# XiaRho/CMDA

Measured on AMD Instinct MI355X. Metric: training images/sec (512x512 image+event, MiT-B5), higher is better.
Workload: dtype bf16

## Files before the change

cmda_amd/_lib.py:

```python
import ctypes
import os

import torch

_HERE = os.path.dirname(os.path.abspath(__file__))
_LIB_PATH = os.environ.get('CMDA_HIP_LIB') or os.path.join(_HERE, 'libcmda_hip.so')

c_i32, c_i64, c_f32, c_vp = ctypes.c_int32, ctypes.c_int64, ctypes.c_float, ctypes.c_void_p

F32, BF16 = 0, 1
U8, I64 = 0, 1
ABI_VERSION, ABI_EXT_VERSION = 8, 1
ABI_EXT2_VERSION = 1
ABI_EXT3_VERSION = 1
ABI_EXT4_VERSION = 1
ABI_EXT5_VERSION = 1


class View(ctypes.Structure):
    _fields_ = [('ptr', c_vp), ('ld', c_i64), ('R', c_i64), ('Cc', c_i64), ('batch_stride', c_i64), ('batch2_stride', c_i64),
                ('conv', c_i32), ('H', c_i32), ('W', c_i32), ('C', c_i32), ('OH', c_i32), ('OW', c_i32),
                ('KH', c_i32), ('KW', c_i32), ('stride', c_i32), ('pad', c_i32), ('dil', c_i32),
                ('in_dil', c_i32), ('reflect', c_i32), ('vec_ok', c_i32)]


class GemmParams(ctypes.Structure):
    _fields_ = [('A', View), ('B', View), ('a_kstrided', c_i32), ('b_kstrided', c_i32), ('C', c_vp),
                ('ldc', c_i64), ('c_batch_stride', c_i64), ('c_batch2_stride', c_i64), ('M', c_i32), ('N', c_i32),
                ('K', c_i32), ('batch', c_i32), ('batch2', c_i32), ('splits', c_i32), ('alpha', c_f32), ('beta', c_f32), ('bias', c_vp),
                ('act', c_i32), ('res', c_vp), ('ldres', c_i64), ('res_batch_stride', c_i64), ('res_batch2_stride', c_i64),
                ('rowscale', c_vp), ('rows_per_scale', c_i32), ('out_f32', c_i32), ('atomic', c_i32),
                ('dtype', c_i32), ('c_vec_ok', c_i32), ('colsum', c_vp),
                ('c_patch_ow', c_i32), ('c_patch_kh', c_i32), ('c_patch_kwci', c_i32), ('tile_hint', c_i32), ('c_perm_ci', c_i32), ('c_perm_cells', c_i32),
                ('res_f32', c_i32), ('colstats_rows', c_i32), ('colstats', c_vp)]


class CmdaError(RuntimeError):
    pass


_ERR = {-1: 'bad shape', -2: 'unsupported dtype', -3: 'HIP launch error', -4: 'unsupported argument combination'}

_lib = None
_emulated = False


def _declare(lib):
    lib.cmda_abi_version.restype = ctypes.c_int
    lib.cmda_layernorm_bwd_ws_floats.restype = ctypes.c_int64
# ... 6 lines not shown
    if not hasattr(lib, 'cmdax_abi_version'):
        raise CmdaError('the kernel library lacks the ABI extension (cmdax_*): rebuild it')
    lib.cmdax_abi_version.restype = ctypes.c_int
    if lib.cmdax_abi_version() != ABI_EXT_VERSION:
        raise CmdaError('libcmda_hip.so ABI extension version mismatch')
    if not hasattr(lib, 'cmdax2_abi_version'):
        raise CmdaError('the kernel library lacks the second ABI table (cmdax2_*): rebuild it')
    lib.cmdax2_abi_version.restype = ctypes.c_int
    if lib.cmdax2_abi_version() != ABI_EXT2_VERSION:
        raise CmdaError('libcmda_hip.so second ABI table (cmdax2_*) version mismatch')
    if not hasattr(lib, 'cmdax3_abi_version'):
        raise CmdaError('the kernel library lacks the third ABI table (cmdax3_*): rebuild it')
    lib.cmdax3_abi_version.restype = ctypes.c_int
    if lib.cmdax3_abi_version() != ABI_EXT3_VERSION:
        raise CmdaError('libcmda_hip.so third ABI table (cmdax3_*) version mismatch')
    lib.cmdax3_sky_mask_ws_bytes.restype = ctypes.c_int64
    lib.cmdax3_sky_mask_ws_bytes.argtypes = [ctypes.c_int, ctypes.c_int, ctypes.c_int]
    if not hasattr(lib, 'cmdax4_abi_version'):
        raise CmdaError('the kernel library lacks the fourth ABI table (cmdax4_*): rebuild it')
    lib.cmdax4_abi_version.restype = ctypes.c_int
    if lib.cmdax4_abi_version() != ABI_EXT4_VERSION:
        raise CmdaError('libcmda_hip.so fourth ABI table (cmdax4_*) version mismatch')
    lib.cmdax4_cow_mask_ws_bytes.restype = ctypes.c_int64
    lib.cmdax4_cow_mask_ws_bytes.argtypes = [ctypes.c_int, ctypes.c_int, ctypes.c_int, ctypes.c_int]
    if not hasattr(lib, 'cmdax5_abi_version'):
        raise CmdaError('the kernel library lacks the fifth ABI table (cmdax5_*): rebuild it')
    lib.cmdax5_abi_version.restype = ctypes.c_int
    if lib.cmdax5_abi_version() != ABI_EXT5_VERSION:
        raise CmdaError('libcmda_hip.so fifth ABI table (cmdax5_*) version mismatch')
    lib.cmdax5_voxel_ordered_ws_bytes.restype = ctypes.c_int64
    lib.cmdax5_voxel_ordered_ws_bytes.argtypes = [ctypes.c_int, ctypes.c_int64, ctypes.c_int, ctypes.c_int, ctypes.c_int]
    lib.cmdax5_events_norm_ws_bytes.restype = ctypes.c_int64
    lib.cmdax5_events_norm_ws_bytes.argtypes = [ctypes.c_int, ctypes.c_int64]
    return lib


def _load():
    global _lib
    if _lib is not None:
        return _lib
    if not os.path.exists(_LIB_PATH):
        raise CmdaError(
            f'{_LIB_PATH} not found: build the gfx950 kernel library first '
            '(python -c "import __graft_entry__ as g; g.build()" or `make hip`). '
            'cmda_amd has no CPU fallback.')
    _lib = _declare(ctypes.CDLL(_LIB_PATH))
    if _lib.cmda_abi_version() != ABI_VERSION:
        raise CmdaError('libcmda_hip.so ABI version mismatch')
    return _lib


def _bind_for_tests(path):
    global _lib, _emulated
    _lib = _declare(ctypes.CDLL(path))
    _emulated = True
    return _lib


def _unbind_for_tests():
    global _lib, _emulated
    _lib = None
    _emulated = False


def emulated():
    return _emulated
# ... 55 lines not shown
```

cmda_amd/csrc/dwconv.hip:

```cpp
#include "common.h"
#include <cstdlib>

namespace {

struct RunGeom {
  int H, W, dil, rpc, rpr;
  long nruns;
};
static inline RunGeom run_geom(int B, int H, int W, int dil, int run) {
  RunGeom g;
  g.H = H; g.W = W; g.dil = dil;
  const int per_class = (W + dil - 1) / dil;
  g.rpc = (per_class + run - 1) / run;
  g.rpr = dil * g.rpc;
  g.nruns = (long)B * H * g.rpr;
  return g;
}

#ifdef CMDA_EMU
#define CMDA_DW_PIN(v) (void)(v)
#else
#define CMDA_DW_PIN(v) asm volatile("" : "+v"(v))
#endif
template <typename T> struct Raw;
template <> struct Raw<float> {
  float4 v;
  __device__ __forceinline__ void load(const float* p, bool ok) {
    v = *reinterpret_cast<const float4*>(p);
    if (!ok) v = make_float4(0.f, 0.f, 0.f, 0.f);
  }
  __device__ __forceinline__ void unpack(float (&o)[4]) const { o[0] = v.x; o[1] = v.y; o[2] = v.z; o[3] = v.w; }
};
template <> struct Raw<bf16_t> {
// ... 275 lines not shown
  for (int r = 0; r < RL; ++r) {
    const int gr = rgrp[r];
    if (gr >= 0) {
      if (g0 < 0) g0 = gr;
      else if (gr != g0) uniform = false;
    }
  }
  if (g0 < 0) return;
  const unsigned slot = (unsigned)blk.by & (CMDA_BN_SLOTS - 1);
  if (uniform) {
    if (py != 0) return;
    float* wsl = stats + ((long)g0 * (CMDA_BN_SLOTS + 1) + slot) * 2 * (long)C + c;
#pragma unroll
    for (int q = 0; q < 4; ++q) {
      float a = 0.f, b2 = 0.f;
#pragma unroll
      for (int r = 0; r < RL; ++r) {
        a += red[r][cx][q];
        b2 += red[r][cx][4 + q];
      }
      atomicAdd(wsl + q, a);
      atomicAdd(wsl + C + q, b2);
    }
  } else if (grp >= 0) {
    float* wsl = stats + ((long)grp * (CMDA_BN_SLOTS + 1) + slot) * 2 * (long)C + c;
#pragma unroll
    for (int q = 0; q < 4; ++q) {
      atomicAdd(wsl + q, cs[q]);
      atomicAdd(wsl + C + q, cq[q]);
    }
  }
}

template <int CQ>
static __device__ __forceinline__ void dw_fold_atomics(float (&red)[256 / CQ][CQ][41], const float (&acc)[9][4], const float (&accb)[4],
                                                       float* __restrict__ dw, float* __restrict__ dbias, int bx, int C) {
  constexpr int RL = 256 / CQ;
  const int cx = threadIdx.x % CQ, py = threadIdx.x / CQ;
  {
    float* slot = red[py][cx];
#pragma unroll
    for (int t = 0; t < 9; ++t)
#pragma unroll
      for (int j = 0; j < 4; ++j) slot[t * 4 + j] = acc[t][j];
#pragma unroll
    for (int j = 0; j < 4; ++j) slot[36 + j] = accb[j];
  }
  __syncthreads();
  for (int k = threadIdx.x; k < CQ * 40; k += blockDim.x) {
    const int gx = k / 40, v = k - gx * 40;
    const int cc = (bx * CQ + gx) * 4;
    if (cc >= C) continue;
    float s = 0.f;
#pragma unroll
    for (int l = 0; l < RL; ++l) s += red[l][gx][v];
    if (v < 36) {
      const int t = v >> 2, j = v & 3;
      atomicAdd(dw + (cc + j) * 9 + t, s);
    } else if (dbias) {
      atomicAdd(dbias + cc + (v - 36), s);
    }
  }
}

template <typename T, int CQ>
__global__ __launch_bounds__(256) void dw_bwd_weight_kernel(const T* __restrict__ dz, const T* __restrict__ x,
// ... 322 lines not shown
  if (npix * C <= 0) return CMDA_OK;
  if ((C & 3) || dil < 1) return CMDA_ERR_SHAPE;
  if (too_big(npix)) return CMDA_ERR_SHAPE;
  const int gx = (C / 4 + 63) / 64;
  if (dil >= 2 && MODE != 1 && (MODE == 2 || act == 0)) {
    DilGeom dg;
    dg.H = H; dg.W = W; dg.dil = dil;
    dg.rpc = ((W + dil - 1) / dil + DRUN - 1) / DRUN;
    dg.nthreads = (long)B * dil * dil * dg.rpc;
    constexpr int cq = 64;
    const long nb = (dg.nthreads + 256 / cq - 1) / (256 / cq) * gx;
    if (too_big(dg.nthreads) || nb > 0x7fffffffL) return CMDA_ERR_SHAPE;
    CMDA_DISPATCH_DTYPE(dtype, CMDA_LAUNCH((dw_dilated_kernel<T, MODE == 1 ? 0 : MODE, cq>), dim3((unsigned)nb), dim3(256), 0, stream,
                                           (const T*)x, w, bias, (T*)out, dg, C, act, accumulate, gx, stats, imgs_per_group));
    CMDA_CHECK_LAUNCH();
  }
  if (stats) return CMDA_ERR_UNSUPPORTED;
  if constexpr (MODE != 1) {
    int band;
    if (walk_takes<MODE>(B, H, W, C, dil, dtype, &band)) {
      const int rc = launch_walk<MODE, 64>(x, w, bias, da, out, nullptr, nullptr, B, H, W, C, act, accumulate, stream, band);
      if (rc != kWalkDeclined) return rc;
    }
  }
  const RunGeom g = run_geom(B, H, W, dil, run_len(dtype));
  if (too_big(g.nruns)) return CMDA_ERR_SHAPE;
  const long nblk = (g.nruns + 3) / 4 * gx;
  if (nblk > 0x7fffffffL) return CMDA_ERR_SHAPE;
  dim3 grid((unsigned)nblk);
  CMDA_DISPATCH_DTYPE(dtype, CMDA_LAUNCH((dw_stencil_kernel<T, MODE>), grid, dim3(256), 0, stream, (const T*)x, w, bias,
                                         (const T*)da, (T*)out, g, C, act, accumulate, gx));
  CMDA_CHECK_LAUNCH();
}
}

extern "C" int cmda_dwconv3x3_fwd(const void* x, const float* w, const float* bias, void* y, int B, int H, int W, int C,
                                  int dil, int act, int dtype, void* stream) {
  return launch_stencil<0>(x, w, bias, nullptr, y, B, H, W, C, dil, act, 0, dtype, stream);
}

extern "C" int cmda_dwconv3x3_fwd_stats(const void* x, const float* w, const float* bias, void* y, int B, int H, int W, int C,
                                        int dil, float* colstats, int imgs_per_group, int dtype, void* stream) {
  if (!colstats || imgs_per_group < 1 || B % imgs_per_group || dil < 2) return CMDA_ERR_UNSUPPORTED;
  return launch_stencil<0>(x, w, bias, nullptr, y, B, H, W, C, dil, 0, 0, dtype, stream, colstats, imgs_per_group);
}

extern "C" int cmda_dwconv3x3_gelu_bwd_prep(const void* x, const float* w, const float* bias, const void* da, void* dz,
                                            int B, int H, int W, int C, int dil, int dtype, void* stream) {
  return launch_stencil<1>(x, w, bias, da, dz, B, H, W, C, dil, 2, 0, dtype, stream);
}

extern "C" int cmda_dwconv3x3_bwd_data(const void* dy, const float* w, void* dx, int B, int H, int W, int C, int dil,
                                       int accumulate, int dtype, void* stream) {
  return launch_stencil<2>(dy, w, nullptr, nullptr, dx, B, H, W, C, dil, 0, accumulate, dtype, stream);
}

extern "C" int cmda_dwconv3x3_bwd_weight(const void* dz, const void* x, float* dw, float* dbias, int B, int H, int W,
                                         int C, int dil, int dtype, void* stream) {
  const long npix = (long)B * H * W;
  if (npix * C <= 0) return CMDA_OK;
  if ((C & 3) || dil < 1) return CMDA_ERR_SHAPE;
  const RunGeom g = run_geom(B, H, W, dil, run_len(dtype));
  if (too_big(npix) || too_big(g.nruns)) return CMDA_ERR_SHAPE;
  constexpr int cq = 16, rl = 256 / cq;
  const int gx = (C / 4 + cq - 1) / cq;
  int k = 8;
// ... 32 lines not shown
```

cmda_amd/decode_heads.py:

```python
import torch
import torch.nn as nn

from . import nn as K
from . import deferred, ops
from . import runtime as rt
from .registry import HEADS, LOSSES, build_loss


class ConvModule(nn.Module):

    def __init__(self, cin, cout, k, padding=0, dilation=1, groups=1, norm=True):
        super().__init__()
        self.conv = nn.Conv2d(cin, cout, k, padding=padding, dilation=dilation, groups=groups, bias=not norm)
        self.bn = nn.BatchNorm2d(cout) if norm else None
        nn.init.kaiming_normal_(self.conv.weight, a=0, mode='fan_out', nonlinearity='relu')
        if self.conv.bias is not None:
            nn.init.zeros_(self.conv.bias)
        self.k, self.padding, self.dilation, self.groups = k, padding, dilation, groups


class DepthwiseSeparableConvModule(nn.Module):
    def __init__(self, cin, cout, k, padding, dilation):
        super().__init__()
        self.depthwise_conv = ConvModule(cin, cin, k, padding=padding, dilation=dilation, groups=cin)
        self.pointwise_conv = ConvModule(cin, cout, 1)


class MLP(nn.Module):
    def __init__(self, input_dim=2048, embed_dim=768):
        super().__init__()
        self.proj = nn.Linear(input_dim, embed_dim)


def _bn_stats_ws(bn, dev, M, C, groups):
    if not bn.training or M % groups or not ops.colstats_ok(M // groups, C):
        return None
    return ops.bn_stats_ws(dev, groups, C)


def _bn_fwd(bn, x, y, M, C, relu, ldy=None, coff=0, groups=1, order=None, stats_ws=None):
    if bn.training:
        mean, rstd = ops.bn_train_fwd(x, bn.weight, bn.bias, y, bn.running_mean, bn.running_var, M // groups, C, bn.eps,
                                      bn.momentum, relu, ldy, coff, groups, order, stats_ws=stats_ws)
    else:
        mean, rstd = bn.running_mean, torch.rsqrt(bn.running_var + bn.eps)
        ops.bn_apply(x, mean, rstd, bn.weight, bn.bias, y, M, C, relu, ldy, coff)
        mean, rstd = mean.expand(groups, C).contiguous(), rstd.expand(groups, C).contiguous()
    return mean, rstd


def _bn_bwd(bn, dy, x, stats, M, C, relu, lddy=None, coff=0, groups=1):
    mean, rstd = stats
    return ops.bn_train_bwd(dy, x, mean, rstd, bn.weight, bn.bias, rt.grad(bn.weight), rt.grad(bn.bias), M // groups, C, relu,
                            lddy, coff, groups)


class ASPPWrapper(nn.Module):

    def __init__(self, in_channels, channels, sep, dilations, pool=False, norm_cfg=None, act_cfg=None,
                 align_corners=False, context_cfg=None):
        super().__init__()
        assert not pool and context_cfg is None, 'only the configuration CMDA uses is implemented'
        assert sep, 'CMDA uses the depthwise-separable ASPP'
        self.dilations = tuple(dilations)
        self.in_channels, self.channels = in_channels, channels
        mods = []
        for d in self.dilations:
            mods.append(ConvModule(in_channels, channels, 1) if d == 1 else
                        DepthwiseSeparableConvModule(in_channels, channels, 3, padding=d, dilation=d))
        self.aspp_modules = nn.ModuleList(mods)
        self.bottleneck = ConvModule(len(self.dilations) * channels, channels, 3, padding=1)

    def fwd(self, x, B, H, W, groups=1, order=None):
        M, Cin, Ch = B * H * W, self.in_channels, self.channels
        nb = len(self.dilations)
        cat = torch.empty(M, nb * Ch, dtype=rt.compute_dtype(), device=x.device)
        saved = []
        g = dict(groups=groups, order=order)
        for j, (d, m) in enumerate(zip(self.dilations, self.aspp_modules)):
            if d == 1:
                ws = _bn_stats_ws(m.bn, x.device, M, Ch, groups)
                z = K.linear_fwd(x, m.conv.weight, None, M, Cin, colstats=None if ws is None else (ws, M // groups))
                st = _bn_fwd(m.bn, z, cat, M, Ch, True, nb * Ch, j * Ch, stats_ws=ws, **g)
                saved.append((z, st))
            else:
                dwm, pwm = m.depthwise_conv, m.pointwise_conv
                ws = _bn_stats_ws(dwm.bn, x.device, M, Cin, groups) if (d >= 2 and B % groups == 0) else None
                u = ops.dwconv_fwd(x, rt.wdw(dwm.conv.weight), None, B, H, W, Cin, d, None, colstats=None if ws is None else (ws, B // groups))
                ub = torch.empty_like(u)
                st_u = _bn_fwd(dwm.bn, u, ub, M, Cin, True, stats_ws=ws, **g)
                ws = _bn_stats_ws(pwm.bn, x.device, M, Ch, groups)
                z = K.linear_fwd(ub, pwm.conv.weight, None, M, Cin, colstats=None if ws is None else (ws, M // groups))
                st_z = _bn_fwd(pwm.bn, z, cat, M, Ch, True, nb * Ch, j * Ch, stats_ws=ws, **g)
                saved.append((u, st_u, ub, z, st_z))
        ws = _bn_stats_ws(self.bottleneck.bn, x.device, M, Ch, groups)
        zb, _, _ = K.conv_fwd(cat, self.bottleneck.conv.weight, None, B, H, W, 1, 1, colstats=None if ws is None else (ws, M // groups))
        feat = torch.empty_like(zb)
        st_b = _bn_fwd(self.bottleneck.bn, zb, feat, M, Ch, True, stats_ws=ws, **g)
        return feat, (x, cat, saved, zb, st_b, groups)

    def bwd(self, sv, dfeat, B, H, W):
        x, cat, saved, zb, st_b, groups = sv
        M, Cin, Ch = B * H * W, self.in_channels, self.channels
        nb = len(self.dilations)
        dzb = _bn_bwd(self.bottleneck.bn, dfeat, zb, st_b, M, Ch, True, groups=groups)
        dcat = K.conv_bwd(dzb, cat, self.bottleneck.conv.weight, None, B, H, W, 1, 1)
        dx = torch.empty(M, Cin, dtype=rt.compute_dtype(), device=x.device)
        first = True
        for j, (d, m) in enumerate(zip(self.dilations, self.aspp_modules)):
            if d == 1:
                z, st = saved[j]
                dz = _bn_bwd(m.bn, dcat, z, st, M, Ch, True, nb * Ch, j * Ch, groups=groups)
                K.linear_bwd(dz, x, m.conv.weight, None, M, Cin, dx_out=dx, dx_beta=0.0 if first else 1.0)
            else:
                u, st_u, ub, z, st_z = saved[j]
                dwm, pwm = m.depthwise_conv, m.pointwise_conv
                dz = _bn_bwd(pwm.bn, dcat, z, st_z, M, Ch, True, nb * Ch, j * Ch, groups=groups)
                dub = K.linear_bwd(dz, ub, pwm.conv.weight, None, M, Cin)
                du = _bn_bwd(dwm.bn, dub, u, st_u, M, Cin, True, groups=groups)
                deferred.tail_defer(lambda du=du, gw=rt.grad(dwm.conv.weight).view(Cin, 9), d=d:
                                    ops.dwconv_bwd_weight(du, x, gw, None, B, H, W, Cin, d))
                ops.dwconv_bwd_data(du, rt.wdw(dwm.conv.weight), B, H, W, Cin, d, out=dx, accumulate=not first)
            first = False
        return dx


def build_layer(in_channels, out_channels, type, **kwargs):
    if type == 'id':
        return nn.Identity()
    if type == 'mlp':
        return MLP(input_dim=in_channels, embed_dim=out_channels)
    if type == 'aspp':
        return ASPPWrapper(in_channels=in_channels, channels=out_channels, **kwargs)
    raise NotImplementedError(type)


@LOSSES.register_module()
class CrossEntropyLoss(nn.Module):

    def __init__(self, use_sigmoid=False, use_mask=False, reduction='mean', class_weight=None, loss_weight=1.0):
        super().__init__()
        assert not use_sigmoid and not use_mask, 'only the softmax cross-entropy of configs/fusion/* is implemented'
        assert reduction == 'mean'
        self.use_sigmoid, self.use_mask, self.reduction = use_sigmoid, use_mask, reduction
        self.loss_weight, self.class_weight = loss_weight, class_weight


def ce_losses_fwd(logits, seg_label, seg_weight, ignore_index, loss_weight):
    B, _, H, W = seg_label.shape
    label = seg_label.view(B, H, W)
    wgt = seg_weight.float().contiguous() if seg_weight is not None else None
    acc, lse = ops.ce_upsample_fwd(logits, label, wgt, H, W, ignore_index)
    n = float(B * H * W)
    loss = acc[0] * (loss_weight / n)
    accuracy = acc[1:2] * (100.0 / n)
# ... 360 lines not shown
```

cmda_amd/ops.py:

```python
import ctypes
import os

import numpy as np
import torch

from . import _lib as L
from . import deferred as D
from ._lib import BF16, F32, GemmParams, View, c_f32, c_i32, c_i64, call, check_dev, dtype_tag, ptr, stream_of

_ESIZE = {torch.float32: 4, torch.bfloat16: 2}


def _chunk(t):
    return 16 // _ESIZE[t.dtype]


def plain_view(t, rows, cols, ld=None, batch_stride=0, offset=0, batch2_stride=0):
    ld = cols if ld is None else ld
    es = _ESIZE[t.dtype]
    ch = 16 // es
    base = t.data_ptr() + offset * es
    vec_ok = int(base % 16 == 0 and ld % ch == 0 and batch_stride % ch == 0 and batch2_stride % ch == 0)
    v = View(ptr=base, ld=ld, R=rows, Cc=cols, batch_stride=batch_stride, batch2_stride=batch2_stride, conv=0,
             vec_ok=vec_ok,
# ... 529 lines not shown
    return y


def dwconv_gelu_bwd_prep(x, w, bias, da, B, H, W, C, dil=1):
    check_dev(x, w, bias, da)
    dz = torch.empty_like(x)
    call('cmda_dwconv3x3_gelu_bwd_prep', ptr(x), ptr(w), ptr(bias), ptr(da), ptr(dz), c_i32(B), c_i32(H), c_i32(W),
         c_i32(C), c_i32(dil), dtype_tag(x), stream_of(x))
    return dz


def dwconv_gelu_bwd_fused(x, w, bias, da, dw, dbias, B, H, W, C, dil=1):
    check_dev(x, w, bias, da, dw, dbias)
    dz = torch.empty_like(x)
    call('cmda_dwconv3x3_gelu_bwd_fused', ptr(x), ptr(w), ptr(bias), ptr(da), ptr(dz), ptr(dw), ptr(dbias), c_i32(B), c_i32(H),
         c_i32(W), c_i32(C), c_i32(dil), dtype_tag(x), stream_of(x))
    return dz


def dwconv_bwd_data(dy, w, B, H, W, C, dil=1, out=None, accumulate=False):
    check_dev(dy, w, out)
    dx = torch.empty_like(dy) if out is None else out
    call('cmda_dwconv3x3_bwd_data', ptr(dy), ptr(w), ptr(dx), c_i32(B), c_i32(H), c_i32(W), c_i32(C), c_i32(dil),
         c_i32(int(accumulate)), dtype_tag(dy), stream_of(dy))
    return dx


def dwconv_bwd_weight(dz, x, dw, dbias, B, H, W, C, dil=1):
    check_dev(dz, x, dw, dbias)
    call('cmda_dwconv3x3_bwd_weight', ptr(dz), ptr(x), ptr(dw), ptr(dbias), c_i32(B), c_i32(H), c_i32(W), c_i32(C),
         c_i32(dil), dtype_tag(x), stream_of(x))


def bilinear_fwd(x, y, B, IH, IW, OH, OW, C, ldy=None, coff=0):
    check_dev(x, y)
    call('cmda_bilinear_fwd', ptr(x), ptr(y), c_i32(B), c_i32(IH), c_i32(IW), c_i32(OH), c_i32(OW), c_i32(C),
         c_i32(C if ldy is None else ldy), c_i32(coff), dtype_tag(x), stream_of(x))
    return y


def bilinear_bwd(dy, dx, B, IH, IW, OH, OW, C, ldy=None, coff=0):
    check_dev(dy, dx)
    call('cmda_bilinear_bwd', ptr(dy), ptr(dx), c_i32(B), c_i32(IH), c_i32(IW), c_i32(OH), c_i32(OW), c_i32(C),
         c_i32(C if ldy is None else ldy), c_i32(coff), dtype_tag(dy), stream_of(dy))
    return dx


BN_FUSED_STATS = os.environ.get('CMDA_BN_FUSED_STATS', '1') != '0'
def bn_stats_ws(device, groups, C):
    if not BN_FUSED_STATS:
        return None
    need = groups * int(L.lib().cmda_bn_ws_floats(C))
    ws = D.workspace('bn', device, need, make_in_capture=False)
    return None if ws is None else ws[:need]


def colstats_ok(rows_per_group, N):
    return BN_FUSED_STATS and rows_per_group > 0 and rows_per_group % 256 == 0 and N % 4 == 0


def bn_train_fwd(x, gamma, beta, y, running_mean, running_var, M, C, eps, momentum, relu, ldy=None, coff=0, groups=1, order=None,
                 stats_ws=None):
    check_dev(x, gamma, beta, y, running_mean, running_var, stats_ws)
    mean = torch.empty(groups, C, dtype=torch.float32, device=x.device)
    rstd = torch.empty(groups, C, dtype=torch.float32, device=x.device)
    ws = stats_ws if stats_ws is not None else torch.empty(groups * L.lib().cmda_bn_ws_floats(C), dtype=torch.float32, device=x.device)
    order_c = (ctypes.c_int * groups)(*order) if order is not None else None
    call('cmda_bn_train_fwd', ptr(x), ptr(gamma), ptr(beta), ptr(y), ptr(mean), ptr(rstd), ptr(running_mean),
         ptr(running_var), ptr(ws), c_i64(M), c_i32(C), c_f32(eps), c_f32(momentum), c_i32(int(relu)),
         c_i32(C if ldy is None else ldy), c_i32(coff), c_i32(groups), order_c, c_i32(int(stats_ws is not None)), dtype_tag(x), stream_of(x))
    return mean, rstd


def bn_train_fwd2(x, gamma, beta, y, M, C, eps, relu, groups=1, res32=None, y2=None, ldy=None, coff=0, stats_ws=None):
    check_dev(x, gamma, beta, y, res32, y2, stats_ws)
    assert res32 is None or res32.dtype == torch.float32
    assert y2 is None or y2.dtype == torch.bfloat16
    mean = torch.empty(groups, C, dtype=torch.float32, device=x.device)
    rstd = torch.empty(groups, C, dtype=torch.float32, device=x.device)
    ws = stats_ws if stats_ws is not None else torch.empty(groups * L.lib().cmda_bn_ws_floats(C), dtype=torch.float32, device=x.device)
    call('cmda_bn_train_fwd2', ptr(x), dtype_tag(x), ptr(gamma), ptr(beta), ptr(y), dtype_tag(y), ptr(mean), ptr(rstd), None, None,
         ptr(ws), c_i64(M), c_i32(C), c_f32(eps), c_f32(0.0), c_i32(int(relu)), c_i32(C if ldy is None else ldy), c_i32(coff),
         c_i32(groups), None, ptr(res32), ptr(y2), c_i32(int(stats_ws is not None)), stream_of(x))
    return mean, rstd


def bn_apply(x, mean, rstd, gamma, beta, y, M, C, relu, ldy=None, coff=0):
# ... 617 lines not shown
```

Measured before the change: 40.42.

## Fuse three dilated ASPP depthwise convs into one shared-input kernel for data grad

Adds a HIP kernel that computes the three dilated depthwise 3x3 convolutions of the ASPP head (dilations d, 2d, 3d) in a single pass. Each thread walks rows of the shared dilation lattice, so input or upstream-gradient loads are reused across the three branches. The backward data-gradient path is enabled by default and replaces three separate kernels that each read and accumulate into dx. The fused forward path is compiled but turned off by a module flag. This adds register pressure and complexity, and it falls back to the per-branch kernels when the shape is unsupported.

After: 40.63 (median of 6 runs). Within noise of the previous version (+0.5%).

```diff
diff --git a/cmda_amd/_lib.py b/cmda_amd/_lib.py
--- a/cmda_amd/_lib.py
+++ b/cmda_amd/_lib.py
@@ -15,6 +15,7 @@
 ABI_EXT3_VERSION = 1
 ABI_EXT4_VERSION = 1
 ABI_EXT5_VERSION = 1
+ABI_EXT6_VERSION = 1
 
 
 class View(ctypes.Structure):
@@ -87,6 +88,13 @@
     lib.cmdax5_voxel_ordered_ws_bytes.argtypes = [ctypes.c_int, ctypes.c_int64, ctypes.c_int, ctypes.c_int, ctypes.c_int]
     lib.cmdax5_events_norm_ws_bytes.restype = ctypes.c_int64
     lib.cmdax5_events_norm_ws_bytes.argtypes = [ctypes.c_int, ctypes.c_int64]
+    if not hasattr(lib, 'cmdax6_abi_version'):
+        raise CmdaError('the kernel library lacks the sixth ABI table (cmdax6_*): rebuild it')
+    lib.cmdax6_abi_version.restype = ctypes.c_int
+    if lib.cmdax6_abi_version() != ABI_EXT6_VERSION:
+        raise CmdaError('libcmda_hip.so sixth ABI table (cmdax6_*) version mismatch')
+    for name in ('cmdax6_dwconv3x3_dil3_fwd_stats', 'cmdax6_dwconv3x3_dil3_bwd_data'):
+        getattr(lib, name).restype = ctypes.c_int
     return lib
 
 
diff --git a/cmda_amd/csrc/dwconv.hip b/cmda_amd/csrc/dwconv.hip
--- a/cmda_amd/csrc/dwconv.hip
+++ b/cmda_amd/csrc/dwconv.hip
@@ -1,4 +1,5 @@
 #include "common.h"
+#include "../../include/cmda_hip_ext6.h"
 #include <cstdlib>
 
 namespace {
@@ -340,6 +341,368 @@
   }
 }
 
+constexpr int D3W = DRUN + 6;
+#ifdef CMDA_EMU
+#define CMDA_D3_FENCE() (void)0
+#else
+#define CMDA_D3_FENCE() __builtin_amdgcn_sched_barrier(0)
+#endif
+static __device__ __forceinline__ float d3_tap(float a, float b, float c) {
+#ifdef CMDA_EMU
+  return c + a * b;
+#else
+  return fmaf(a, b, c);
+#endif
+}
+template <typename T> struct Raw2;
+template <> struct Raw2<float> {
+  float2 v;
+  __device__ __forceinline__ void zero() { v.x = v.y = 0.f; }
+  __device__ __forceinline__ void pin() {}
+  __device__ __forceinline__ void load(const char* p) { v = *reinterpret_cast<const float2*>(p); }
+  __device__ __forceinline__ void unpack(float (&o)[2]) const { o[0] = v.x; o[1] = v.y; }
+  static __device__ __forceinline__ void store(char* p, const float (&o)[2]) {
+    float2 t;
+    t.x = o[0]; t.y = o[1];
+    *reinterpret_cast<float2*>(p) = t;
+  }
+};
+template <> struct Raw2<bf16_t> {
+  unsigned v;
+  __device__ __forceinline__ void zero() { v = 0u; }
+  __device__ __forceinline__ void pin() { CMDA_DW_PIN(v); }
+  __device__ __forceinline__ void load(const char* p) { v = *reinterpret_cast<const unsigned*>(p); }
+  __device__ __forceinline__ void unpack(float (&o)[2]) const {
+    o[0] = __uint_as_float(v << 16);
+    o[1] = __uint_as_float(v & 0xffff0000u);
+  }
+  static __device__ __forceinline__ void store(char* p, const float (&o)[2]) {
+    *reinterpret_cast<unsigned*>(p) = (unsigned)f2bf(o[0]) | ((unsigned)f2bf(o[1]) << 16);
+  }
+};
+struct Dil3Geom {
+  int H, W, g, rpc;
+  long nthreads;
+};
+constexpr int D3CQ = 64;
+constexpr int D3WS = D3CQ * 2;
+static __device__ __forceinline__ void dil3_stage_taps(float (&wl)[27 * D3WS], const float* __restrict__ w1, const float* __restrict__ w2,
+                                                       const float* __restrict__ w3, int c0, int C, bool mirror) {
+  for (int e = threadIdx.x; e < 27 * D3WS; e += 256) {
+    const int tp = e / D3WS, cc = c0 + e % D3WS;
+    const int kk = tp / 9, t9 = tp % 9;
+    const float* w = kk == 0 ? w1 : kk == 1 ? w2 : w3;
+    wl[e] = cc < C ? w[(mirror ? 8 - t9 : t9) * C + cc] : 0.f;
+  }
+  __syncthreads();
+}
+template <typename T, bool ACC>
+static __device__ __forceinline__ void dw_dil3_dgrad_walk(const T* __restrict__ du1, const T* __restrict__ du2, const T* __restrict__ du3,
+                                                          const float* wl, unsigned wo0, T* __restrict__ dx, const Dil3Geom& g, int C,
+                                                          int c, unsigned tu) {
+  const int k = (int)(tu % (unsigned)g.rpc);
+  const unsigned t1 = tu / (unsigned)g.rpc;
+  const int rho_w = (int)(t1 % (unsigned)g.g);
+  const unsigned t2 = t1 / (unsigned)g.g;
+  const int rho_h = (int)(t2 % (unsigned)g.g), b = (int)(t2 / (unsigned)g.g);
+  const int nr = (g.H - rho_h + g.g - 1) / g.g;
+  const int ncol = (g.W - rho_w + g.g - 1) / g.g;
+  const int k0 = k * DRUN;
+  if (nr <= 0 || k0 >= ncol) return;
+  const unsigned pixb = (unsigned)C * (unsigned)sizeof(T);
+  const unsigned rowb = (unsigned)g.W * pixb;
+  const unsigned rb0 = (unsigned)(b * g.H + rho_h) * rowb, rstep = (unsigned)g.g * rowb;
+  unsigned coff[D3W];
+  bool cok[D3W];
+#pragma unroll
+  for (int ci = 0; ci < D3W; ++ci) {
+    const int kc = k0 - 3 + ci;
+    cok[ci] = kc >= 0 && kc < ncol;
+    coff[ci] = (unsigned)(rho_w + (cok[ci] ? kc : k0) * g.g) * pixb + (unsigned)c * (unsigned)sizeof(T);
+  }
+  const char* ub[3] = {reinterpret_cast<const char*>(du1), reinterpret_cast<const char*>(du2), reinterpret_cast<const char*>(du3)};
+  char* ob = reinterpret_cast<char*>(dx);
+
+  Raw2<T> cur[3][D3W], nxt[3][D3W], pcur[DRUN], pnxt[DRUN];
+  const unsigned rblast = rb0 + (unsigned)(nr - 1) * rstep;
+  auto request = [&](int r, unsigned rb, Raw2<T> (&dst)[3][D3W], Raw2<T> (&pdst)[DRUN]) {
+    const unsigned rbq = r < nr ? rb : rblast;
+#pragma unroll
+    for (int kk = 0; kk < 3; ++kk)
+#pragma unroll
+      for (int ci = 2 - kk; ci <= DRUN + 3 + kk; ++ci) dst[kk][ci].load(ub[kk] + (rbq + coff[ci]));
+    if (ACC) {
+      const unsigned rbp = (r >= 3 && r - 3 < nr) ? rb - 3u * rstep : rb0;
+#pragma unroll
+      for (int i = 0; i < DRUN; ++i) pdst[i].load(ob + (rbp + coff[i + 3]));
+    }
+  };
+  float acc[7][DRUN][2];
+#pragma unroll
+  for (int sl = 0; sl < 7; ++sl)
+#pragma unroll
+    for (int i = 0; i < DRUN; ++i) acc[sl][i][0] = acc[sl][i][1] = 0.f;
+  request(0, rb0, cur, pcur);
+  unsigned rbn = rb0 + rstep;
+  const int nt = nr + 3;
+  for (int t0 = 0; t0 < nt; t0 += 7) {
+#pragma unroll
+    for (int s = 0; s < 7; ++s) {
+      const int t = t0 + s;
+      if (t < nt) {
+        CMDA_DW_PIN(rbn);
+        request(t + 1, rbn, nxt, pnxt);
+        if (t < nr) {
+          unsigned wo = wo0;
+          CMDA_DW_PIN(wo);
+#pragma unroll
+          for (int kk = 0; kk < 3; ++kk) {
+            float in[D3W][2];
+#pragma unroll
+            for (int ci = 2 - kk; ci <= DRUN + 3 + kk; ++ci) {
+              if (cok[ci]) cur[kk][ci].unpack(in[ci]);
+              else in[ci][0] = in[ci][1] = 0.f;
+            }
+#pragma unroll
+            for (int kh = 0; kh < 3; ++kh) {
+              const int sl = (s + (1 - kh) * (kk + 1) + 7) % 7;
+#pragma unroll
+              for (int kw = 0; kw < 3; ++kw) {
+                const float* wt = wl + (kk * 9 + kh * 3 + kw) * D3WS + wo;
+                const float wv[2] = {wt[0], wt[1]};
+#pragma unroll
+                for (int i = 0; i < DRUN; ++i)
+#pragma unroll
+                  for (int q = 0; q < 2; ++q) acc[sl][i][q] = d3_tap(in[i + 3 + (kw - 1) * (kk + 1)][q], wv[q], acc[sl][i][q]);
+              }
+              CMDA_D3_FENCE();
+            }
+          }
+        }
+        const int so = (s + 4) % 7;
+        if (t >= 3) {
+          const unsigned rbo = rbn - 4u * rstep;
+#pragma unroll
+          for (int i = 0; i < DRUN; ++i) {
+            if (k0 + i < ncol) {
+              float o[2] = {acc[so][i][0], acc[so][i][1]};
+              if (ACC) {
+                float p[2];
+                pcur[i].unpack(p);
+                o[0] += p[0];
+                o[1] += p[1];
+              }
+              Raw2<T>::store(ob + (rbo + coff[i + 3]), o);
+            }
+          }
+        }
+#pragma unroll
+        for (int i = 0; i < DRUN; ++i) acc[so][i][0] = acc[so][i][1] = 0.f;
+#pragma unroll
+        for (int kk = 0; kk < 3; ++kk)
+#pragma unroll
+          for (int ci = 2 - kk; ci <= DRUN + 3 + kk; ++ci) cur[kk][ci] = nxt[kk][ci];
+#pragma unroll
+        for (int i = 0; i < DRUN; ++i) pcur[i] = pnxt[i];
+        rbn += rstep;
+      }
+    }
+  }
+}
+
+template <typename T, bool ACC>
+__global__ __launch_bounds__(256, 2) void dw_dil3_dgrad_kernel(const T* __restrict__ du1, const T* __restrict__ du2, const T* __restrict__ du3,
+                                                            const float* __restrict__ w1, const float* __restrict__ w2,
+                                                            const float* __restrict__ w3, T* __restrict__ dx, Dil3Geom g, int C, int gx) {
+  constexpr int CQ = D3CQ;
+  __shared__ float wl[27 * D3WS];
+  const int cx = threadIdx.x % CQ, py = threadIdx.x / CQ;
+  const BlockXY blk = xcd_block(gx);
+  const int c = (blk.bx * CQ + cx) * 2;
+  const long t = blk.by * (256 / CQ) + py;
+  dil3_stage_taps(wl, w1, w2, w3, blk.bx * CQ * 2, C, true);
+  if (c < C && t < g.nthreads) dw_dil3_dgrad_walk<T, ACC>(du1, du2, du3, wl, (unsigned)cx * 2, dx, g, C, c, (unsigned)t);
+}
+
+template <typename T>
+static __device__ __forceinline__ void dw_dil3_fwd_walk(const T* __restrict__ x, const float* wl, unsigned wo0, T* __restrict__ u1, T* __restrict__ u2,
+                                                        T* __restrict__ u3, const Dil3Geom& g, int C, int c, unsigned tu, bool do_stats,
+                                                        int imgs_per_group, float (&cs)[3][2], float (&cq)[3][2], int& grp) {
+  const int k = (int)(tu % (unsigned)g.rpc);
+  const unsigned t1 = tu / (unsigned)g.rpc;
+  const int rho_w = (int)(t1 % (unsigned)g.g);
+  const unsigned t2 = t1 / (unsigned)g.g;
+  const int rho_h = (int)(t2 % (unsigned)g.g), b = (int)(t2 / (unsigned)g.g);
+  const int nr = (g.H - rho_h + g.g - 1) / g.g;
+  const int ncol = (g.W - rho_w + g.g - 1) / g.g;
+  const int k0 = k * DRUN;
+  if (nr <= 0 || k0 >= ncol) return;
+  if (do_stats) grp = b / imgs_per_group;
+  const unsigned pixb = (unsigned)C * (unsigned)sizeof(T);
+  const unsigned rowb = (unsigned)g.W * pixb;
+  const unsigned rb0 = (unsigned)(b * g.H + rho_h) * rowb, rstep = (unsigned)g.g * rowb;
+  unsigned coff[D3W];
+  bool cok[D3W];
+#pragma unroll
+  for (int ci = 0; ci < D3W; ++ci) {
+    const int kc = k0 - 3 + ci;
+    cok[ci] = kc >= 0 && kc < ncol;
+    coff[ci] = (unsigned)(rho_w + (cok[ci] ? kc : k0) * g.g) * pixb + (unsigned)c * (unsigned)sizeof(T);
+  }
+  const char* xb = reinterpret_cast<const char*>(x);
+  char* ob[3] = {reinterpret_cast<char*>(u1), reinterpret_cast<char*>(u2), reinterpret_cast<char*>(u3)};
+
+  Raw2<T> ring[8][D3W];
+  auto request = [&](int r, unsigned rb, Raw2<T> (&dst)[D3W]) {
+    if (r < nr) {
+#pragma unroll
+      for (int ci = 0; ci < D3W; ++ci) dst[ci].load(xb + (rb + coff[ci]));
+    } else {
+#pragma unroll
+      for (int ci = 0; ci < D3W; ++ci) dst[ci].zero();
+    }
+  };
+#pragma unroll
+  for (int sl = 4; sl < 8; ++sl)
+#pragma unroll
+    for (int ci = 0; ci < D3W; ++ci) ring[sl][ci].zero();
+  request(0, rb0, ring[0]);
+  request(1, rb0 + rstep, ring[1]);
+  request(2, rb0 + 2u * rstep, ring[2]);
+  request(3, rb0 + 3u * rstep, ring[3]);
+  unsigned rb = rb0;
+  for (int j0 = 0; j0 < nr; j0 += 8) {
+#pragma unroll
+    for (int s = 0; s < 8; ++s) {
+      const int j = j0 + s;
+      if (j < nr) {
+        CMDA_DW_PIN(rb);
+        request(j + 4, rb + 4u * rstep, ring[(s + 4) % 8]);
+        unsigned wo = wo0;
+        CMDA_DW_PIN(wo);
+#pragma unroll
+        for (int a = -2; a <= 3; ++a)
+#pragma unroll
+          for (int ci = 0; ci < D3W; ++ci) ring[(s + a + 8) % 8][ci].pin();
+#pragma unroll
+        for (int kk = 0; kk < 3; ++kk) {
+          float acc[DRUN][2];
+#pragma unroll
+          for (int i = 0; i < DRUN; ++i) acc[i][0] = acc[i][1] = 0.f;
+#pragma unroll
+          for (int kh = 0; kh < 3; ++kh) {
+            const int sl = (s + (kh - 1) * (kk + 1) + 8) % 8;
+            float in[D3W][2];
+#pragma unroll
+            for (int ci = 2 - kk; ci <= DRUN + 3 + kk; ++ci) {
+              if (cok[ci]) ring[sl][ci].unpack(in[ci]);
+              else in[ci][0] = in[ci][1] = 0.f;
+            }
+#pragma unroll
+            for (int kw = 0; kw < 3; ++kw) {
+              const float* wt = wl + (kk * 9 + kh * 3 + kw) * D3WS + wo;
+              const float wv[2] = {wt[0], wt[1]};
+#pragma unroll
+              for (int i = 0; i < DRUN; ++i)
+#pragma unroll
+                for (int q = 0; q < 2; ++q) acc[i][q] = d3_tap(in[i + 3 + (kw - 1) * (kk + 1)][q], wv[q], acc[i][q]);
+            }
+            CMDA_D3_FENCE();
+          }
+#pragma unroll
+          for (int i = 0; i < DRUN; ++i) {
+            if (k0 + i < ncol) {
+              Raw2<T>::store(ob[kk] + (rb + coff[i + 3]), acc[i]);
+              if (do_stats) {
+#pragma unroll
+                for (int q = 0; q < 2; ++q) {
+                  cs[kk][q] += acc[i][q];
+                  cq[kk][q] += acc[i][q] * acc[i][q];
+                }
+              }
+            }
+          }
+        }
+        rb += rstep;
+      }
+    }
+  }
+}
+
+template <typename T>
+__global__ __launch_bounds__(256, 2) void dw_dil3_fwd_kernel(const T* __restrict__ x, const float* __restrict__ w1, const float* __restrict__ w2,
+                                                          const float* __restrict__ w3, T* __restrict__ u1, T* __restrict__ u2,
+                                                          T* __restrict__ u3, Dil3Geom g, int C, int gx, float* __restrict__ st1,
+                                                          float* __restrict__ st2, float* __restrict__ st3, int imgs_per_group) {
+  constexpr int CQ = D3CQ;
+  const int cx = threadIdx.x % CQ, py = threadIdx.x / CQ;
+  const BlockXY blk = xcd_block(gx);
+  const int c = (blk.bx * CQ + cx) * 2;
+  const long t = blk.by * (256 / CQ) + py;
+  const bool do_stats = st1 != nullptr;
+  float cs[3][2] = {{0.f, 0.f}, {0.f, 0.f}, {0.f, 0.f}}, cq[3][2] = {{0.f, 0.f}, {0.f, 0.f}, {0.f, 0.f}};
+  int grp = -1;
+  __shared__ float wl[27 * D3WS];
+  dil3_stage_taps(wl, w1, w2, w3, blk.bx * CQ * 2, C, false);
+  if (c < C && t < g.nthreads)
+    dw_dil3_fwd_walk<T>(x, wl, (unsigned)cx * 2, u1, u2, u3, g, C, c, (unsigned)t, do_stats, imgs_per_group, cs, cq, grp);
+  if (!do_stats) return;
+  constexpr int RL = 256 / CQ;
+  __shared__ float red[RL][CQ][12];
+  __shared__ int rgrp[RL];
+  if (cx == 0) rgrp[py] = grp;
+#pragma unroll
+  for (int kk = 0; kk < 3; ++kk)
+#pragma unroll
+    for (int q = 0; q < 2; ++q) {
+      red[py][cx][kk * 4 + q] = cs[kk][q];
+      red[py][cx][kk * 4 + 2 + q] = cq[kk][q];
+    }
+  __syncthreads();
+  if (c >= C) return;
+  bool uniform = true;
+  int g0 = -1;
+#pragma unroll
+  for (int r = 0; r < RL; ++r) {
+    const int gr = rgrp[r];
+    if (gr >= 0) {
+      if (g0 < 0) g0 = gr;
+      else if (gr != g0) uniform = false;
+    }
+  }
+  if (g0 < 0) return;
+  const unsigned slot = (unsigned)blk.by & (CMDA_BN_SLOTS - 1);
+  float* const st[3] = {st1, st2, st3};
+  if (uniform) {
+    if (py != 0) return;
+#pragma unroll
+    for (int kk = 0; kk < 3; ++kk) {
+      float* wsl = st[kk] + ((long)g0 * (CMDA_BN_SLOTS + 1) + slot) * 2 * (long)C + c;
+#pragma unroll
+      for (int q = 0; q < 2; ++q) {
+        float a = 0.f, b2 = 0.f;
+#pragma unroll
+        for (int r = 0; r < RL; ++r) {
+          a += red[r][cx][kk * 4 + q];
+          b2 += red[r][cx][kk * 4 + 2 + q];
+        }
+        atomicAdd(wsl + q, a);
+        atomicAdd(wsl + C + q, b2);
+      }
+    }
+  } else if (grp >= 0) {
+#pragma unroll
+    for (int kk = 0; kk < 3; ++kk) {
+      float* wsl = st[kk] + ((long)grp * (CMDA_BN_SLOTS + 1) + slot) * 2 * (long)C + c;
+#pragma unroll
+      for (int q = 0; q < 2; ++q) {
+        atomicAdd(wsl + q, cs[kk][q]);
+        atomicAdd(wsl + C + q, cq[kk][q]);
+      }
+    }
+  }
+}
+
 template <int CQ>
 static __device__ __forceinline__ void dw_fold_atomics(float (&red)[256 / CQ][CQ][41], const float (&acc)[9][4], const float (&accb)[4],
                                                        float* __restrict__ dw, float* __restrict__ dbias, int bx, int C) {
@@ -728,6 +1091,58 @@
                                          (const T*)da, (T*)out, g, C, act, accumulate, gx));
   CMDA_CHECK_LAUNCH();
 }
+
+static inline int dil3_geom(int B, int H, int W, int C, int d1, int d2, int d3, int dtype, Dil3Geom* dg, int* gx, long* nb, int cq) {
+  if (B < 1 || H < 1 || W < 1 || C < 1 || (C & 3) || d1 < 1 || d2 != 2 * d1 || d3 != 3 * d1) return CMDA_ERR_SHAPE;
+  if (dtype != CMDA_F32 && dtype != CMDA_BF16) return CMDA_ERR_DTYPE;
+  const long bytes = (long)B * H * W * C * (dtype == CMDA_BF16 ? 2 : 4);
+  if (bytes >= (1L << 32)) return CMDA_ERR_SHAPE;
+  dg->H = H; dg->W = W; dg->g = d1;
+  dg->rpc = ((W + d1 - 1) / d1 + DRUN - 1) / DRUN;
+  dg->nthreads = (long)B * d1 * d1 * dg->rpc;
+  *gx = (C / 2 + cq - 1) / cq;
+  *nb = (dg->nthreads + 256 / cq - 1) / (256 / cq) * *gx;
+  if (too_big(dg->nthreads) || *nb > 0x7fffffffL) return CMDA_ERR_SHAPE;
+  return CMDA_OK;
+}
+}
+
+extern "C" int cmdax6_abi_version(void) { return 1; }
+
+extern "C" int cmdax6_dwconv3x3_dil3_fwd_stats(const void* x, const float* w1, const float* w2, const float* w3, void* u1, void* u2,
+                                               void* u3, int B, int H, int W, int C, int d1, int d2, int d3, float* st1, float* st2,
+                                               float* st3, int imgs_per_group, int dtype, void* stream) {
+  constexpr int cq = D3CQ;
+  Dil3Geom dg;
+  int gx;
+  long nb;
+  const int rc = dil3_geom(B, H, W, C, d1, d2, d3, dtype, &dg, &gx, &nb, cq);
+  if (rc != CMDA_OK) return rc;
+  if (!x || !w1 || !w2 || !w3 || !u1 || !u2 || !u3) return CMDA_ERR_UNSUPPORTED;
+  const bool stats = st1 || st2 || st3;
+  if (stats && (!st1 || !st2 || !st3 || imgs_per_group < 1 || B % imgs_per_group)) return CMDA_ERR_UNSUPPORTED;
+  CMDA_DISPATCH_DTYPE(dtype, CMDA_LAUNCH((dw_dil3_fwd_kernel<T>), dim3((unsigned)nb), dim3(256), 0, stream, (const T*)x, w1, w2, w3,
+                                         (T*)u1, (T*)u2, (T*)u3, dg, C, gx, st1, st2, st3, stats ? imgs_per_group : 1));
+  CMDA_CHECK_LAUNCH();
+}
+
+extern "C" int cmdax6_dwconv3x3_dil3_bwd_data(const void* du1, const void* du2, const void* du3, const float* w1, const float* w2,
+                                              const float* w3, void* dx, int B, int H, int W, int C, int d1, int d2, int d3,
+                                              int accumulate, int dtype, void* stream) {
+  constexpr int cq = D3CQ;
+  Dil3Geom dg;
+  int gx;
+  long nb;
+  const int rc = dil3_geom(B, H, W, C, d1, d2, d3, dtype, &dg, &gx, &nb, cq);
+  if (rc != CMDA_OK) return rc;
+  if (!du1 || !du2 || !du3 || !w1 || !w2 || !w3 || !dx) return CMDA_ERR_UNSUPPORTED;
+  if (accumulate)
+    CMDA_DISPATCH_DTYPE(dtype, CMDA_LAUNCH((dw_dil3_dgrad_kernel<T, true>), dim3((unsigned)nb), dim3(256), 0, stream, (const T*)du1,
+                                           (const T*)du2, (const T*)du3, w1, w2, w3, (T*)dx, dg, C, gx));
+  else
+    CMDA_DISPATCH_DTYPE(dtype, CMDA_LAUNCH((dw_dil3_dgrad_kernel<T, false>), dim3((unsigned)nb), dim3(256), 0, stream, (const T*)du1,
+                                           (const T*)du2, (const T*)du3, w1, w2, w3, (T*)dx, dg, C, gx));
+  CMDA_CHECK_LAUNCH();
 }
 
 extern "C" int cmda_dwconv3x3_fwd(const void* x, const float* w, const float* bias, void* y, int B, int H, int W, int C,
diff --git a/cmda_amd/decode_heads.py b/cmda_amd/decode_heads.py
--- a/cmda_amd/decode_heads.py
+++ b/cmda_amd/decode_heads.py
@@ -1,3 +1,5 @@
+import os
+
 import torch
 import torch.nn as nn
 
@@ -53,6 +55,10 @@
     mean, rstd = stats
     return ops.bn_train_bwd(dy, x, mean, rstd, bn.weight, bn.bias, rt.grad(bn.weight), rt.grad(bn.bias), M // groups, C, relu,
                             lddy, coff, groups)
+
+
+ASPP_DIL3_FWD = False
+ASPP_DIL3_BWD = True
 
 
 class ASPPWrapper(nn.Module):
@@ -71,13 +77,38 @@
         self.aspp_modules = nn.ModuleList(mods)
         self.bottleneck = ConvModule(len(self.dilations) * channels, channels, 3, padding=1)
 
+    def _dil3(self, on):
+        if not on or os.environ.get('CMDA_ASPP_DIL3', '1') == '0':
+            return None
+        js = [j for j, d in enumerate(self.dilations) if d != 1]
+        if len(js) != 3 or js[2] - js[0] != 2:
+            return None
+        d1, d2, d3 = (self.dilations[j] for j in js)
+        return js if d1 >= 2 and d2 == 2 * d1 and d3 == 3 * d1 else None
+
+    def _dil3_fwd(self, js, x, B, H, W, groups):
+        M, Cin, Ch = B * H * W, self.in_channels, self.channels
+        dws = [self.aspp_modules[j].depthwise_conv for j in js]
+        wss = None
+        if (B % groups == 0 and Ch <= Cin and all(m.bn.training for m in dws) and M % groups == 0
+                and ops.colstats_ok(M // groups, Cin)):
+            wss = ops.bn_stats_ws_n(x.device, groups, Cin, 3)
+        us = ops.dwconv_dil3_fwd(x, [rt.wdw(m.conv.weight) for m in dws], B, H, W, Cin, [self.dilations[j] for j in js],
+                                 colstats=None if wss is None else (wss, B // groups))
+        if us is None:
+            return {}
+        return {j: (u, None if wss is None else wss[i]) for i, (j, u) in enumerate(zip(js, us))}
+
     def fwd(self, x, B, H, W, groups=1, order=None):
         M, Cin, Ch = B * H * W, self.in_channels, self.channels
         nb = len(self.dilations)
         cat = torch.empty(M, nb * Ch, dtype=rt.compute_dtype(), device=x.device)
         saved = []
         g = dict(groups=groups, order=order)
+        js, fused = self._dil3(ASPP_DIL3_FWD), {}
         for j, (d, m) in enumerate(zip(self.dilations, self.aspp_modules)):
+            if js is not None and j == js[0]:
+                fused = self._dil3_fwd(js, x, B, H, W, groups)
             if d == 1:
                 ws = _bn_stats_ws(m.bn, x.device, M, Ch, groups)
                 z = K.linear_fwd(x, m.conv.weight, None, M, Cin, colstats=None if ws is None else (ws, M // groups))
@@ -85,8 +116,12 @@
                 saved.append((z, st))
             else:
                 dwm, pwm = m.depthwise_conv, m.pointwise_conv
-                ws = _bn_stats_ws(dwm.bn, x.device, M, Cin, groups) if (d >= 2 and B % groups == 0) else None
-                u = ops.dwconv_fwd(x, rt.wdw(dwm.conv.weight), None, B, H, W, Cin, d, None, colstats=None if ws is None else (ws, B // groups))
+                if j in fused:
+                    u, ws = fused.pop(j)
+                else:
+                    ws = _bn_stats_ws(dwm.bn, x.device, M, Cin, groups) if (d >= 2 and B % groups == 0) else None
+                    u = ops.dwconv_fwd(x, rt.wdw(dwm.conv.weight), None, B, H, W, Cin, d, None,
+                                       colstats=None if ws is None else (ws, B // groups))
                 ub = torch.empty_like(u)
                 st_u = _bn_fwd(dwm.bn, u, ub, M, Cin, True, stats_ws=ws, **g)
                 ws = _bn_stats_ws(pwm.bn, x.device, M, Ch, groups)
@@ -107,6 +142,7 @@
         dcat = K.conv_bwd(dzb, cat, self.bottleneck.conv.weight, None, B, H, W, 1, 1)
         dx = torch.empty(M, Cin, dtype=rt.compute_dtype(), device=x.device)
         first = True
+        js, dus = self._dil3(ASPP_DIL3_BWD), []
         for j, (d, m) in enumerate(zip(self.dilations, self.aspp_modules)):
             if d == 1:
                 z, st = saved[j]
@@ -120,7 +156,17 @@
                 du = _bn_bwd(dwm.bn, dub, u, st_u, M, Cin, True, groups=groups)
                 deferred.tail_defer(lambda du=du, gw=rt.grad(dwm.conv.weight).view(Cin, 9), d=d:
                                     ops.dwconv_bwd_weight(du, x, gw, None, B, H, W, Cin, d))
-                ops.dwconv_bwd_data(du, rt.wdw(dwm.conv.weight), B, H, W, Cin, d, out=dx, accumulate=not first)
+                if js is not None:
+                    dus.append((du, rt.wdw(dwm.conv.weight), d))
+                    if j != js[-1]:
+                        continue
+                    if ops.dwconv_dil3_bwd_data([t[0] for t in dus], [t[1] for t in dus], B, H, W, Cin, [t[2] for t in dus],
+                                                out=dx, accumulate=not first) is None:
+                        for du_k, w_k, d_k in dus:
+                            ops.dwconv_bwd_data(du_k, w_k, B, H, W, Cin, d_k, out=dx, accumulate=not first)
+                            first = False
+                else:
+                    ops.dwconv_bwd_data(du, rt.wdw(dwm.conv.weight), B, H, W, Cin, d, out=dx, accumulate=not first)
             first = False
         return dx
 
diff --git a/cmda_amd/ops.py b/cmda_amd/ops.py
--- a/cmda_amd/ops.py
+++ b/cmda_amd/ops.py
@@ -585,6 +585,38 @@
          c_i32(dil), dtype_tag(x), stream_of(x))
 
 
+_ERR_SHAPE = -1
+
+
+def _dil3_call(name, *args):
+    rc = getattr(L.lib(), name)(*args)
+    if rc == _ERR_SHAPE:
+        return False
+    if rc != 0:
+        raise L.CmdaError(f'{name} failed: {L._ERR.get(rc, rc)}')
+    return True
+
+
+def dwconv_dil3_fwd(x, ws, B, H, W, C, dils, colstats=None):
+    check_dev(x, *ws)
+    st = (None, None, None) if colstats is None else colstats[0]
+    check_dev(*st)
+    us = [torch.empty_like(x) for _ in range(3)]
+    ok = _dil3_call('cmdax6_dwconv3x3_dil3_fwd_stats', ptr(x), ptr(ws[0]), ptr(ws[1]), ptr(ws[2]), ptr(us[0]), ptr(us[1]), ptr(us[2]),
+                    c_i32(B), c_i32(H), c_i32(W), c_i32(C), c_i32(dils[0]), c_i32(dils[1]), c_i32(dils[2]), ptr(st[0]), ptr(st[1]),
+                    ptr(st[2]), c_i32(1 if colstats is None else colstats[1]), dtype_tag(x), stream_of(x))
+    return tuple(us) if ok else None
+
+
+def dwconv_dil3_bwd_data(dus, ws, B, H, W, C, dils, out=None, accumulate=False):
+    check_dev(*dus, *ws, out)
+    dx = torch.empty_like(dus[0]) if out is None else out
+    ok = _dil3_call('cmdax6_dwconv3x3_dil3_bwd_data', ptr(dus[0]), ptr(dus[1]), ptr(dus[2]), ptr(ws[0]), ptr(ws[1]), ptr(ws[2]), ptr(dx),
+                    c_i32(B), c_i32(H), c_i32(W), c_i32(C), c_i32(dils[0]), c_i32(dils[1]), c_i32(dils[2]), c_i32(int(accumulate)),
+                    dtype_tag(dus[0]), stream_of(dus[0]))
+    return dx if ok else None
+
+
 def bilinear_fwd(x, y, B, IH, IW, OH, OW, C, ldy=None, coff=0):
     check_dev(x, y)
     call('cmda_bilinear_fwd', ptr(x), ptr(y), c_i32(B), c_i32(IH), c_i32(IW), c_i32(OH), c_i32(OW), c_i32(C),
@@ -606,6 +638,14 @@
     need = groups * int(L.lib().cmda_bn_ws_floats(C))
     ws = D.workspace('bn', device, need, make_in_capture=False)
     return None if ws is None else ws[:need]
+
+
+def bn_stats_ws_n(device, groups, C, n):
+    if not BN_FUSED_STATS:
+        return None
+    need = groups * int(L.lib().cmda_bn_ws_floats(C))
+    ws = D.workspace('bn', device, n * need, make_in_capture=False)
+    return None if ws is None else tuple(ws[k * need:(k + 1) * need] for k in range(n))
 
 
 def colstats_ok(rows_per_group, N):
diff --git a/include/cmda_hip_ext6.h b/include/cmda_hip_ext6.h
--- /dev/null
+++ b/include/cmda_hip_ext6.h
@@ -0,0 +1,22 @@
+#ifndef CMDA_HIP_EXT6_H
+#define CMDA_HIP_EXT6_H
+#include "cmda_hip_ext5.h"
+
+#ifdef __cplusplus
+extern "C" {
+#endif
+
+int cmdax6_abi_version(void);
+
+int cmdax6_dwconv3x3_dil3_fwd_stats(const void* x, const float* w1, const float* w2, const float* w3, void* u1, void* u2, void* u3,
+                                    int B, int H, int W, int C, int d1, int d2, int d3, float* st1, float* st2, float* st3,
+                                    int imgs_per_group, int dtype, void* stream);
+
+int cmdax6_dwconv3x3_dil3_bwd_data(const void* du1, const void* du2, const void* du3, const float* w1, const float* w2,
+                                   const float* w3, void* dx, int B, int H, int W, int C, int d1, int d2, int d3, int accumulate,
+                                   int dtype, void* stream);
+
+#ifdef __cplusplus
+}
+#endif
+#endif
```
